# librosa/librosa

Measured on AMD Instinct MI355X. Metric: STFT+mel frames/sec (n_fft=2048 hop=512), higher is better.
Workload: dtype f32

## Files before the change

### librosa_amd/csrc/lra_api.hip

```cpp
#include <dlfcn.h>
#include <hip/hip_runtime.h>
#include <rocfft/rocfft.h>

#include <algorithm>
#include <atomic>
#include <chrono>
#include <cmath>
#include <cstdio>
#include <cstdlib>
#include <cstring>
#include <map>
#include <memory>
#include <mutex>
#include <string>
#include <thread>
#include <vector>

#include "../../include/librosa_amd.h"
#ifndef LRA_ISTFT16_DEFAULT
#define LRA_ISTFT16_DEFAULT 0
#endif
#ifndef LRA_V3_DEFAULT
#define LRA_V3_DEFAULT 1
#endif
// ... 46 lines not shown
    int opt_stft_iters = 0;
    int opt_istft_strip_groups = 0;
    int opt_variant = -1;
    int opt_autotune = 1;
    int opt_mel_runs = 1;
    int opt_mel_tile = 0;
    int opt_generic_mel = 0;
    int opt_lds_pad = 0;
    int opt_v2 = 1;
    int opt_istft16 = LRA_ISTFT16_DEFAULT;
    int opt_placement_retry = 0;
    struct PlacedAlloc {
        size_t padded = 0;
        std::vector<hipMemGenericAllocationHandle_t> handles;
        bool plain = false;
    };
    std::map<void*, PlacedAlloc> placed;
    std::mutex placed_mu;
    std::vector<std::pair<void*, size_t>> placed_retired;
    size_t placed_va_spent = 0;
    static constexpr size_t kPlacedVaBudget = (size_t)4 << 40;
    double placed_best_gbps = 0.0;
    int opt_v3 = LRA_V3_DEFAULT;
    int opt_mel_pc = LRA_MEL_PC_DEFAULT;
    int opt_mel_many = 1;
    int opt_cqt_merge = 1;
    int opt_hpss_tile = 1;
    int opt_mixed_inv_pow2 = 1;
    int opt_mixed_pow2_mel = 1;
    int opt_ola4 = 1;
    int opt_mixed_irfft = 1;
    int opt_mixed = 1;
    int opt_direct = 1;
    int opt_xcd_remap = 1;
    unsigned int* d_flag = nullptr;
    std::map<std::pair<int, int>, std::pair<void*, void*>> cqt_tw;
    std::string name;
    struct HostPipe* pipe = nullptr;
    hipStream_t side_stream = nullptr;
    hipStream_t side_main = nullptr;
    static constexpr int kForkRing = 16;
    hipEvent_t fork_event[kForkRing] = {}, side_passed[kForkRing] = {};
    bool fork_used[kForkRing] = {};
    int fork_next = 0;
    static constexpr int kJoinRing = 8;
    hipEvent_t join_event[kJoinRing] = {}, main_passed[kJoinRing] = {};
// ... 193 lines not shown
    if (it != cache.end()) return it->second;
    int per_cu = 0;
    if (lds > 65536) (void)hipFuncSetAttribute(kern, hipFuncAttributeMaxDynamicSharedMemorySize, lds);
    if (hipOccupancyMaxActiveBlocksPerMultiprocessor(&per_cu, kern, block, lds) != hipSuccess) per_cu = 0;
    (void)hipGetLastError();
    cache[key] = per_cu;
    return per_cu;
}

template <class T> struct StftLaunch {
    StftArgs<T> a;
    int mode = 0;
    long long batch = 0;
    int iters_opt = 0;
    int mel_tile_opt = 0;
    int n_cu = 256;
    void* out = nullptr;
    int lds_pad = 0;
    bool xcd_remap = true;
    bool use_v2 = true;
    bool use_direct = true;
    bool mel_v2 = false;
    bool mel_pc = false;
    bool mel_runs = true;
    const lra_mel_plan* mel = nullptr;
    hipStream_t stream = nullptr;
    hipError_t err = hipSuccess;

    template <class Cfg, int MODE> void launch(int shared_bytes) {
        static_assert(Cfg::P <= 4, "at most four Stockham passes are wired up");
        const int lds_probe_v1 = Cfg::FPB * stft_slot_bytes<Cfg>(MODE, a.n_mels, mel_tile_opt > 0 ? mel_tile_opt : 4) + shared_bytes + lds_pad;
        void (*kern)(StftArgs<T>, const T*, void*) = nullptr;
        bool direct = false;
        if constexpr (Cfg::PLAN == 0) {
        kern = stft_kernel<Cfg, MODE, POW_TWO, 0>;
        if (MODE != OUT_COMPLEX && a.power_mode == POW_ONE) kern = stft_kernel<Cfg, MODE, POW_ONE, 0>;
        if (MODE != OUT_COMPLEX && a.power_mode == POW_GENERAL) kern = stft_kernel<Cfg, MODE, POW_GENERAL, 0>;
        if constexpr (sizeof(T) == 4) {
#ifndef LRA_MEL_RA
#define LRA_MEL_RA 1
#endif
            if (ring_rows_aligned<Cfg>(a.hop) && (LRA_MEL_RA || MODE == OUT_COMPLEX || MODE == OUT_POWER)) {
                kern = stft_kernel<Cfg, MODE, POW_TWO, 1>;
                if (MODE != OUT_COMPLEX && a.power_mode == POW_ONE) kern = stft_kernel<Cfg, MODE, POW_ONE, 1>;
                if (MODE != OUT_COMPLEX && a.power_mode == POW_GENERAL) kern = stft_kernel<Cfg, MODE, POW_GENERAL, 1>;
            }
// ... 66 lines not shown
        if (lds > 160 * 1024) { err = hipErrorInvalidValue; return; }
        if (lds > 65536) {
            err = hipFuncSetAttribute(reinterpret_cast<const void*>(kern), hipFuncAttributeMaxDynamicSharedMemorySize, lds);
            if (err != hipSuccess) return;
        }
        a.n_blocks = (int)grid;
        a.xcd_chunk = (xcd_remap && grid >= 64) ? (int)((grid + 7) / 8) : 0;
        const long long launch_grid = a.xcd_chunk ? 8LL * a.xcd_chunk : grid;
        hipLaunchKernelGGL(kern, dim3((unsigned)launch_grid), dim3(Cfg::NT), lds, stream, a, a.y, out);
        err = hipGetLastError();
    }

    template <class Cfg> void launch_pc(int hd) {
        using PL = PcLayout<Cfg>;
        void (*kern)(StftArgs<T>, const T*, void*) = nullptr;
#define LRA_PICKP(HD)                                                        \
    kern = stft_pc_kernel<Cfg, HD, POW_TWO>;                                 \
    if (a.power_mode == POW_ONE) kern = stft_pc_kernel<Cfg, HD, POW_ONE>;    \
    if (a.power_mode == POW_GENERAL) kern = stft_pc_kernel<Cfg, HD, POW_GENERAL>;
        if (hd == 4) { LRA_PICKP(4) } else { LRA_PICKP(8) }
#undef LRA_PICKP
        const int lds = PL::BYTES + lds_pad;
        constexpr int fpb = PL::NP;
        int iters = iters_opt;
        if (iters <= 0) {
            const int per_cu = resident_workgroups(reinterpret_cast<const void*>(kern), PL::NT, lds);
            const long long conc = (long long)n_cu * (per_cu > 0 ? per_cu : 1);
            int best_iters = 0;
            double best_fill = -1.0;
            for (int cand = 176; cand >= 24; --cand) {
                const int wgpc = (a.n_frames + fpb * cand - 1) / (fpb * cand);
                const int it = (a.n_frames + fpb * wgpc - 1) / (fpb * wgpc);
                const double rounds = (double)(batch * wgpc) / (double)conc;
                const double fill = (rounds <= 1.0 && rounds >= 0.6) ? 1.0 : rounds / std::ceil(rounds);
                if (fill > best_fill + 0.02) { best_fill = fill; best_iters = it; }
            }
            iters = best_iters;
            while (iters > 4 && batch * ((a.n_frames + fpb * iters - 1) / (fpb * iters)) < 2LL * n_cu) iters /= 2;
        }
        if (iters < 1) iters = 1;
        a.rot_uniform = 0;
        a.mel_tile = 1;
        a.frames_per_wg = fpb * iters;
        a.wg_per_clip = (a.n_frames + a.frames_per_wg - 1) / a.frames_per_wg;
        a.slot_bytes = PL::FRAME;
        a.shared_off = 0;
        const long long grid = batch * a.wg_per_clip;
        if (grid > 0x7ffffff0LL) { err = hipErrorInvalidConfiguration; return; }
        a.n_blocks = (int)grid;
        a.xcd_chunk = (xcd_remap && grid >= 64) ? (int)((grid + 7) / 8) : 0;
        const long long launch_grid = a.xcd_chunk ? 8LL * a.xcd_chunk : grid;
        hipLaunchKernelGGL(kern, dim3((unsigned)launch_grid), dim3(PL::NT), lds, stream, a, a.y, out);
        err = hipGetLastError();
    }

    template <class Cfg> void operator()() {
        if constexpr (Cfg::REV) {
            err = hipErrorInvalidValue;
            return;
        } else if constexpr (Cfg::PLAN == 1) {
            if (!use_v2 || v2_hop_divisor<Cfg>(a.hop) == 0) { err = hipErrorInvalidValue; return; }
            if (mode == OUT_COMPLEX) launch<Cfg, OUT_COMPLEX>(0);
            else if (mode == OUT_POWER) launch<Cfg, OUT_POWER>(0);
            else if (mode == OUT_MEL2 && mel_pc && mel && mel->melr2_ok && mel_runs) {
                if constexpr (pc_cfg_ok<Cfg>()) {
                    const int hd_pc = v2_hop_divisor<Cfg>(a.hop);
                    if (!pc_bank_ok<Cfg>(a.n_mels, mel->melr2_pmax) || !pc_fits_budget<Cfg>(hd_pc, a.power_mode)) { err = hipErrorInvalidValue; return; }
                    a.melr_w = (const T*)mel->d_melr2_w;
                    a.melr_keep = (const T*)mel->d_melr2_keep;
                    a.melr_addr = mel->d_melr2_addr;
                    a.melr_zero = mel->melr2_zero;
                    a.melr_mid = mel->melr2_mid;
// ... 560 lines not shown
        L.out = out;
        L.a.power_mode = power_mode_of(power);
        L.a.power = (T)power;
        if (mel) {
            L.a.mel_c0 = mel->d_c0;
            L.a.mel_len = mel->d_len;
            L.a.mel_off = mel->d_off;
            L.a.mel_val = (const T*)mel->d_val;
            L.a.n_mels = mel->n_mels;
            L.a.mel_wAB = (const T*)mel->d_wAB;
            L.mel = mel;
        }
        L.a.nonfinite_flag = ctx->d_flag;
        L.mode = (mode == OUT_MEL && mel && mel->two_slope && !ctx->opt_generic_mel) ? OUT_MEL2 : mode;
        L.batch = batch;
        L.stream = ctx->stream;
        L.iters_opt = ctx->opt_stft_iters;
        L.n_cu = ctx->n_cu;
        L.mel_tile_opt = ctx->opt_mel_tile;
        L.lds_pad = ctx->opt_lds_pad;
        L.xcd_remap = ctx->opt_xcd_remap != 0;
        L.use_v2 = ctx->opt_v2 != 0;
        L.mel_pc = ctx->opt_mel_pc != 0;
        L.use_direct = ctx->opt_direct != 0;
        L.mel_runs = ctx->opt_mel_runs != 0;
        int variant = ctx->opt_variant >= 0 ? ctx->opt_variant : 0;
        auto launch = [&](int v) -> int {
            StftLaunch<T> Lv = L;
            Lv.a.tw = (const cx<T>*)p->d_tw[v];
            if (!dispatch_logm<T>(p->logm, v, Lv)) return fail(LRA_EINVAL, "unsupported power-of-two size");
            if (Lv.err != hipSuccess) return fail(LRA_EHIP, std::string("stft kernel launch: ") + hipGetErrorString(Lv.err));
            return LRA_OK;
        };
        bool v2_applies = false;
        if constexpr (sizeof(T) == 4)
            v2_applies = ctx->opt_v2 && (L.mode == OUT_COMPLEX || L.mode == OUT_POWER) && p->logm == 10 && v2_hop_divisor<typename CfgSel<float, 10, 0>::type>(p->hop) > 0;
        if (ctx->opt_variant < 0 && ctx->opt_autotune && sizeof(T) == 4 && p->logm == 10 && !v2_applies) {
            int& tuned = p->tuned_variant[L.mode & 3];
            if (tuned < 0 && batch * n_frames >= 65536) LRA_TRY(autotune_variant(ctx, launch, &tuned));
            if (tuned >= 0) variant = tuned;
        }
        bool pc_g = false;
        if constexpr (sizeof(T) == 4) {
            using C6 = typename CfgSel<float, 10, 6>::type;
            if (L.mode == OUT_MEL2 && ctx->opt_mel_pc == 2 && p->logm == 10 && mel && mel->melr2_ok && ctx->opt_mel_runs && ctx->opt_v2 && (ctx->opt_variant < 0 || ctx->opt_variant == 6))
                pc_g = pc_bank_ok<C6>(mel->n_mels, mel->melr2_pmax) && pc_fits_budget<C6>(v2_hop_divisor<C6>(p->hop), power_mode_of(power));
// ... 672 lines not shown
        return LRA_OK;
    }
    return fail(LRA_EINVAL, "lra_ctx_side: mode must be LRA_SIDE_FORK, LRA_SIDE_BACK, LRA_SIDE_JOIN or LRA_SIDE_END");
}

int lra_ctx_sync(lra_ctx* ctx) {
    LRA_BIND(ctx);
    LRA_HIP(hipStreamSynchronize(ctx->stream));
    return LRA_OK;
}

int lra_ctx_set_option(lra_ctx* ctx, const char* key, int value) {
    if (!ctx || !key) return fail(LRA_EINVAL, "null argument");
    if (!std::strcmp(key, "stft_iters")) ctx->opt_stft_iters = value;
    else if (!std::strcmp(key, "istft_strip_groups")) ctx->opt_istft_strip_groups = value;
    else if (!std::strcmp(key, "mel_tile")) ctx->opt_mel_tile = value;
    else if (!std::strcmp(key, "ablate")) (void)value;
    else if (!std::strcmp(key, "generic_mel")) ctx->opt_generic_mel = value;
    else if (!std::strcmp(key, "pipe_chunk_mb")) ctx->opt_pipe_chunk_mb = value > 0 ? value : 128;
    else if (!std::strcmp(key, "pipe_threads")) ctx->opt_pipe_threads = value > 0 ? value : 1;
    else if (!std::strcmp(key, "lds_pad")) ctx->opt_lds_pad = value;
    else if (!std::strcmp(key, "xcd_remap")) ctx->opt_xcd_remap = value != 0;
    else if (!std::strcmp(key, "v2")) ctx->opt_v2 = value != 0;
    else if (!std::strcmp(key, "mel_pc")) ctx->opt_mel_pc = (value == 1 || value == 2) ? value : 0;
    else if (!std::strcmp(key, "istft16")) ctx->opt_istft16 = value != 0;
    else if (!std::strcmp(key, "placement_retry")) ctx->opt_placement_retry = value < 0 ? 0 : (value > 8 ? 8 : value);
    else if (!std::strcmp(key, "v3")) ctx->opt_v3 = (value == 1 || value == 2) ? value : 0;
    else if (!std::strcmp(key, "cqt_merge")) ctx->opt_cqt_merge = value < 0 ? 0 : (value > 2 ? 2 : (int)value);
    else if (!std::strcmp(key, "mel_many")) ctx->opt_mel_many = value != 0;
    else if (!std::strcmp(key, "direct")) ctx->opt_direct = value != 0;
    else if (!std::strcmp(key, "mixed")) ctx->opt_mixed = value == 2 ? 2 : (value != 0);
    else if (!std::strcmp(key, "hpss_tile")) ctx->opt_hpss_tile = value != 0;
    else if (!std::strcmp(key, "mixed_pow2_mel")) ctx->opt_mixed_pow2_mel = value != 0;
    else if (!std::strcmp(key, "ola4")) ctx->opt_ola4 = value != 0;
    else if (!std::strcmp(key, "mixed_irfft")) ctx->opt_mixed_irfft = value != 0;
    else if (!std::strcmp(key, "mixed_inv_pow2")) ctx->opt_mixed_inv_pow2 = value != 0;
    else if (!std::strcmp(key, "autotune")) ctx->opt_autotune = value != 0;
    else if (!std::strcmp(key, "mel_runs")) ctx->opt_mel_runs = value != 0;
    else if (!std::strcmp(key, "variant")) ctx->opt_variant = (value >= 0 && value < kNumVariants) ? value : -1;
    else return fail(LRA_EINVAL, std::string("unknown option ") + key);
    return LRA_OK;
}

int lra_ctx_nonfinite_reset(lra_ctx* ctx) {
    LRA_BIND(ctx);
    LRA_HIP(hipMemsetAsync(ctx->d_flag, 0, sizeof(unsigned int), ctx->stream));
// ... 1763 lines not shown
```

### librosa_amd/csrc/lra_common.h

```cpp
#pragma once

#include <cstddef>
#include <cstdint>

#ifdef LRA_HOSTSIM
#include <cmath>
#include <cstdio>
#include <cstdlib>
#include <cstring>
#include <vector>
#define LRA_HD inline
#define LRA_UNROLL _Pragma("GCC unroll 64")
#else
#include <hip/hip_runtime.h>
#define LRA_HD __host__ __device__ __forceinline__
#define LRA_UNROLL _Pragma("unroll")
#endif

#ifndef LRA_NO_EXPECT
#define LRA_LIKELY(x) __builtin_expect(!!(x), 1)
#define LRA_UNLIKELY(x) __builtin_expect(!!(x), 0)
#else
#define LRA_LIKELY(x) (x)
#define LRA_UNLIKELY(x) (x)
// ... 248 lines not shown
};
inline State& state() { static thread_local State s; return s; }
}

struct Lds {
    size_t base;
};
template <class V> inline V lds_ld(Lds l, int byte_off) {
    auto& s = sim::state();
    s.note_read(l.base + byte_off, sizeof(V));
    V v; std::memcpy(&v, s.mem.data() + l.base + byte_off, sizeof(V)); return v;
}
template <class V> inline void lds_st(Lds l, int byte_off, V v) {
    auto& s = sim::state();
    s.note_write(l.base + byte_off, sizeof(V));
    std::memcpy(s.mem.data() + l.base + byte_off, &v, sizeof(V));
}
inline Lds lds_sub(Lds l, int byte_off) { Lds r; r.base = l.base + byte_off; return r; }

#define LRA_LAUNDER(p) ((void)0)
#define LRA_ATOMIC_OR(ptr, v) (*(ptr) |= (v))
#define LRA_UNIFORM(x) (x)
#define LRA_KEEP(x) ((void)0)
#define LRA_RAW_TID(tid) (tid)
template <class T> inline T fast_div(T x, T w) { return x / w; }
template <class V> inline void stream_store(V* p, V v) { *p = v; }
template <class V> inline void stream_store16(V* p, V v) { *p = v; }
template <class V> inline V stream_load(const V* p) { return *p; }
template <class T> inline void store4_unaligned(T* p, T a, T b, T c, T d) { p[0] = a; p[1] = b; p[2] = c; p[3] = d; }
#define LRA_PHASE(NT, tid) for (int tid = 0; tid < (NT); ++tid) { ::lra::sim::state().cur_tid = tid;
#define LRA_PHASE_END } ::lra::sim::state().barrier();
#define LRA_PHASE_END_SYNC(WAVE) } ::lra::sim::state().barrier(WAVE);
#define LRA_REGS(Type, name, NT) std::vector<Type> name##_all(NT)
#define LRA_R(name) name##_all[tid]
#define LRA_HALF_SWAP8(name, tid, first, active)                                                                  \
    if ((tid & 63) < 32 && (active)) {                                                                            \
        for (int m_ = 0; m_ < 8; ++m_) std::swap(name##_all[tid].v[(first) + m_], name##_all[tid + 32].v[(first) + m_]); \
    }

#else

struct Lds {
    char* base;
};
#ifndef LRA_LDS_NOMERGE
#define LRA_LDS_NOMERGE 1
#endif
template <class V> LRA_HD V lds_ld(Lds l, int byte_off) {
#if LRA_LDS_NOMERGE
    if constexpr (sizeof(V) == 8) {
        typedef float f2v __attribute__((ext_vector_type(2)));
        const f2v t = *(const volatile __attribute__((address_space(3))) f2v*)(l.base + byte_off);
        return __builtin_bit_cast(V, t);
    }
#endif
    return *reinterpret_cast<const V*>(l.base + byte_off);
}
template <class V> LRA_HD void lds_st(Lds l, int byte_off, V v) { *reinterpret_cast<V*>(l.base + byte_off) = v; }
LRA_HD Lds lds_sub(Lds l, int byte_off) { Lds r; r.base = l.base + byte_off; return r; }

#define LRA_LAUNDER(p) asm volatile("" : "+s"(p))
#define LRA_ATOMIC_OR(ptr, v) atomicOr((ptr), (v))
#define LRA_UNIFORM(x) __builtin_amdgcn_readfirstlane(x)
#define LRA_KEEP(x) asm volatile("" : "+v"(x))
#define LRA_RAW_TID(tid) ((int)threadIdx.x)
__device__ __forceinline__ float fast_div(float x, float w) { return x * __builtin_amdgcn_rcpf(w); }
__device__ __forceinline__ double fast_div(double x, double w) { return x / w; }
#ifndef LRA_NT_STORE
#define LRA_NT_STORE 0
#endif
template <class V> __device__ __forceinline__ void stream_store(V* p, V v) {
#if LRA_NT_STORE
    if constexpr (sizeof(V) == 8) {
        typedef float f2v __attribute__((ext_vector_type(2)));
        __builtin_nontemporal_store(__builtin_bit_cast(f2v, v), reinterpret_cast<f2v*>(p));
    } else if constexpr (sizeof(V) == 16) {
        typedef double d2v __attribute__((ext_vector_type(2)));
        __builtin_nontemporal_store(__builtin_bit_cast(d2v, v), reinterpret_cast<d2v*>(p));
    } else {
        __builtin_nontemporal_store(v, p);
    }
#else
    *p = v;
#endif
}
template <class T> __device__ __forceinline__ void store4_unaligned(T* p, T a, T b, T c, T d) {
    if constexpr (sizeof(T) == 4) {
// ... 77 lines not shown
```

### librosa_amd/csrc/lra_fused.h

```cpp
#pragma once

#include <hip/hip_runtime.h>

#include "lra_dispatch.h"
#include "lra_kernels_pc.h"

template <class Cfg, int MODE, int PM, int RA>
__global__ __launch_bounds__(Cfg::NT, Cfg::MIN_WAVES) void stft_kernel(lra::StftArgs<typename Cfg::real> a, const typename Cfg::real* __restrict__ y,
                                                                     void* __restrict__ out) {
    extern __shared__ __attribute__((aligned(16))) char lra_smem[];
    lra::Lds lds;
    lds.base = lra_smem;
    a.y = y;
    a.D = static_cast<typename Cfg::cplx*>(out);
    a.S = static_cast<typename Cfg::real*>(out);
    a.Mel = static_cast<typename Cfg::real*>(out);
    const int blk = lra::xcd_block((int)blockIdx.x, a.xcd_chunk);
    if (blk >= a.n_blocks) return;
    lra::stft_block<Cfg, MODE, PM, RA>(a, blk, lds);
}

#ifndef LRA_V3_WAVES
#define LRA_V3_WAVES 3
#endif
template <class Cfg, int HD, int MODE, int PM>
__global__ __launch_bounds__(Cfg::NT, (Cfg::NT > 256 ? 1 : (Cfg::TF == 64 && HD >= 4 && PM != lra::POW_GENERAL && MODE != lra::OUT_MELR ? (Cfg::PLAN == 1 ? LRA_V3_WAVES : 3) : 2))) void stft2_kernel(lra::StftArgs<typename Cfg::real> a, const typename Cfg::real* __restrict__ y,
                                                                                  void* __restrict__ out) {
    extern __shared__ __attribute__((aligned(16))) char lra_smem[];
    lra::Lds lds;
    lds.base = lra_smem;
    a.y = y;
    a.D = static_cast<typename Cfg::cplx*>(out);
    a.S = static_cast<typename Cfg::real*>(out);
    a.Mel = static_cast<typename Cfg::real*>(out);
    const int blk = lra::xcd_block((int)blockIdx.x, a.xcd_chunk);
    if (blk >= a.n_blocks) return;
    lra::stft_block2<Cfg, HD, MODE, PM>(a, blk, lds);
}

template <class Cfg, int HD, int PM>
__global__ __launch_bounds__(lra::PcLayout<Cfg>::NT, 3) void stft_pc_kernel(lra::StftArgs<typename Cfg::real> a, const typename Cfg::real* __restrict__ y, void* __restrict__ out) {
    extern __shared__ __attribute__((aligned(16))) char lra_smem[];
    lra::Lds lds;
    lds.base = lra_smem;
    a.y = y;
    a.Mel = static_cast<typename Cfg::real*>(out);
    const int blk = lra::xcd_block((int)blockIdx.x, a.xcd_chunk);
    if (blk >= a.n_blocks) return;
    lra::stft_pc_block<Cfg, HD, PM>(a, blk, lds);
}

template <class Cfg, int HC>
__global__ __launch_bounds__(Cfg::NT, Cfg::MIN_WAVES) void istft_kernel(lra::IstftArgs<typename Cfg::real> a, const typename Cfg::cplx* __restrict__ D,
                                                                      const typename Cfg::real* __restrict__ wss, typename Cfg::real* __restrict__ y) {
    extern __shared__ __attribute__((aligned(16))) char lra_smem[];
    lra::Lds lds;
    lds.base = lra_smem;
    a.D = D;
    a.wss = wss;
    a.y = y;
    const int blk = lra::xcd_block((int)blockIdx.x, a.xcd_chunk);
    if (blk >= a.n_blocks) return;
    lra::istft_block<Cfg, HC>(a, blk, lds);
}


namespace lra {

#define LRA_CFG_ALIAS(NAME, ...) using NAME = typename CfgSel<__VA_ARGS__>::type; using NAME##_mel = typename MelCfgOf<NAME>::type; using NAME##_melmany = typename MelManyCfgOf<NAME>::type;
LRA_CFG_ALIAS(cfg_f32_4, float, 4, 0)
LRA_CFG_ALIAS(cfg_f32_5, float, 5, 0)
// ... 85 lines not shown
```

### librosa_amd/csrc/lra_kernels.h

```cpp
#pragma once

#ifndef LRA_ABLATE
#define LRA_ABLATE 0
#endif

#include <cmath>
#include <limits>

#include "lra_fft.h"

#if defined(LRA_PHASE_TIMER) && !defined(LRA_HOSTSIM)
__device__ unsigned long long lra_phase_ticks[16];
#define LRA_TICK(i)                                                    \
    do {                                                               \
        const unsigned long long now__ = __builtin_amdgcn_s_memtime(); \
        tick_acc[i] += now__ - tick_prev;                              \
        tick_prev = now__;                                             \
    } while (0)
#define LRA_TICK_DECL unsigned long long tick_acc[16] = {}, tick_prev = __builtin_amdgcn_s_memtime()
#define LRA_TICK_FLUSH                                                                    \
    do {                                                                                  \
        if ((threadIdx.x & 63) == 0)                                                      \
            for (int i__ = 0; i__ < 16; ++i__) atomicAdd(&lra_phase_ticks[i__], tick_acc[i__]); \
    } while (0)
// ... 26 lines not shown
    cx<T>* D;
    T* S;
    long long row_pitch;
    T* Mel;
    int power_mode;
    T power;
    const int* mel_c0;
    const int* mel_len;
    const int* mel_off;
    const T* mel_val;
    int n_mels;
    const T* mel_wAB;
    const int* mel_run;
    const int* mel_segd;
    int mel_nyq;
    const T* melr_w;
    const T* melr_keep;
    const int* melr_addr;
    int rot_uniform;
    int melr_pmax;
    int melr_zero, melr_mid;
    int shared_off;
    int n_blocks, xcd_chunk;
    unsigned int* nonfinite_flag;
};

LRA_HD int xcd_block(int b, int chunk) { return chunk > 0 ? (b & 7) * chunk + (b >> 3) : b; }

template <class Cfg> LRA_HD int slot_of(int tid) {
    if (Cfg::FPB == 1) return 0;
    if (Cfg::TF >= 64) return LRA_UNIFORM((int)((unsigned)tid / (unsigned)Cfg::TF));
    return (int)((unsigned)tid / (unsigned)Cfg::TF);
}
template <class Cfg> LRA_HD int lane_of(int tid) { return (int)((unsigned)tid % (unsigned)Cfg::TF); }

#ifndef LRA_MELR_NB_SMALL
#define LRA_MELR_NB_SMALL 4
#endif
#ifndef LRA_MELR_PH_SMALL
#define LRA_MELR_PH_SMALL 3
#endif
constexpr int melr_nb_of_tf(int tf, bool many = false) { return tf >= 32 ? 2 : (many ? 8 : LRA_MELR_NB_SMALL); }
constexpr int melr_ph_of_tf(int tf, bool many = false) { return tf >= 32 ? 4 : (many ? 1 : LRA_MELR_PH_SMALL); }
template <class Cfg> constexpr bool melr_many() { return Cfg::TF == 16 && Cfg::NT == 128; }
template <class Cfg> constexpr int melr_nb() { return melr_nb_of_tf(Cfg::TF, melr_many<Cfg>()); }
template <class Cfg> constexpr int melr_ph() { return melr_ph_of_tf(Cfg::TF, melr_many<Cfg>()); }
// ... 1752 lines not shown
```

### librosa_amd/csrc/lra_kernels_pc.h

```cpp
#pragma once

#include "lra_kernels2.h"

namespace lra {

#ifndef LRA_PC_PRIO_PA
#define LRA_PC_PRIO_PA 3
#endif
#ifndef LRA_PC_PRIO_PS
#define LRA_PC_PRIO_PS 2
#endif
#ifndef LRA_PC_PRIO_CA
#define LRA_PC_PRIO_CA 0
#endif
#ifndef LRA_PC_PRIO_CB
#define LRA_PC_PRIO_CB 1
#endif
#ifndef LRA_PC_ROTATE
#define LRA_PC_ROTATE 1
#endif
#ifndef LRA_PC_SPIN_LIMIT
#define LRA_PC_SPIN_LIMIT (1 << 22)
#endif

// ... 79 lines not shown
    __builtin_amdgcn_fence(__ATOMIC_ACQUIRE, "wavefront");
}
__device__ __forceinline__ int pc_flag_load(Lds l, int off) { return *(const volatile __attribute__((address_space(3))) int*)(l.base + off); }
__device__ __forceinline__ void pc_flag_store(Lds l, int off, int v) { *(volatile __attribute__((address_space(3))) int*)(l.base + off) = v; }
__device__ __forceinline__ void pc_wait(Lds l, int off, int want, unsigned int* sticky) {
    int spins = 0;
    while (true) {
        const int v = LRA_UNIFORM(pc_flag_load(l, off));
        if (LRA_LIKELY(v >= want)) break;
        if (LRA_UNLIKELY(++spins > LRA_PC_SPIN_LIMIT)) {
            if (sticky && (threadIdx.x & 63) == 0) atomicOr(sticky, 2u);
            break;
        }
        __builtin_amdgcn_s_sleep(2);
    }
    pc_fence();
}
__device__ __forceinline__ void pc_wait_ready(Lds l, int off, int want, unsigned int* sticky) {
    if (LRA_UNLIKELY(LRA_UNIFORM(pc_flag_load(l, off)) < want)) pc_wait(l, off, want, sticky);
    else pc_fence();
}
#endif

template <class Cfg, int HD> LRA_HD void pc_producer_prologue(const StftArgs<typename Cfg::real>& a, int clip, int frame0, int tf, Regs2<Cfg, HD>& rg) {
    using T = typename Cfg::real;
    if constexpr (Cfg::PLAN == 1) v3_hoist<Cfg, HD>(rg, tf, a.win, a.tw, a.twr);
    else v2_hoist<Cfg, HD>(rg, tf, a.win, a.tw, a.twr);
    v2_fill<Cfg, HD>(a, clip, frame0, tf, rg);
    if constexpr (v2_rotate_asm_ok<Cfg, HD>() && LRA_PC_ROTATE) {
        LRA_UNROLL
        for (int e = 0; e < Cfg::R; ++e) { LRA_KEEP(rg.raw[e].x); LRA_KEEP(rg.raw[e].y); }
    }
    LRA_UNROLL
    for (int e = 0; e < Regs2<Cfg, HD>::NEW; ++e) rg.pf[e] = mk<T>((T)0, (T)0);
}
template <class Cfg, int HD> LRA_HD void pc_producer_pass0(const StftArgs<typename Cfg::real>& a, int clip, int frame, int it, bool more, int tf, Regs2<Cfg, HD>& rg, Lds fr) {
    if (v2_rotate_asm_ok<Cfg, HD>() && LRA_PC_ROTATE) {
        v2_window_rotating<Cfg, HD>(it, rg);
        if (more) v2_issue_loads<Cfg, HD>(a, clip, frame + 1, tf, rg);
        v2_pass0_dft<Cfg, HD>(tf, rg, fr);
    } else {
        if (it > 0) v2_shift<Cfg, HD>(rg);
        if (more) v2_issue_loads<Cfg, HD>(a, clip, frame + 1, tf, rg);
        v2_pass0<Cfg, HD>(frame < a.n_frames, tf, rg, fr);
    }
}

template <class Cfg, int p> LRA_HD void pc_mid_dft_write(typename Cfg::cplx* v, const typename Cfg::cplx* treg, Lds fr, int tf) {
    if constexpr (Cfg::PLAN == 1) {
        v3_mid_twiddle_dft<Cfg>(v, treg);
        v3_mid_write<Cfg>(v, fr, tf);
    } else {
        pass_twiddle_dft_reg<Cfg, p>(v, treg);
        pass_write<Cfg, p>(v, fr, tf);
    }
}
template <class Cfg, int HD> LRA_HD void pc_last_read(Regs2<Cfg, HD>& rg, Lds fr, int tf) {
    if constexpr (Cfg::PLAN == 1) v3_last_read<Cfg, HD>(rg, fr, tf);
    else v2_last_read<Cfg, HD>(rg, fr, tf);
}
template <class Cfg, int HD, int PM> LRA_HD void pc_last_power_row(const StftArgs<typename Cfg::real>& a, int clip, int frame, int tf, Regs2<Cfg, HD>& rg, Lds pwr) {
    if constexpr (Cfg::PLAN == 1) v3_last_split_store<Cfg, HD, OUT_MELR, PM, false>(a, clip, frame, frame < a.n_frames, tf, rg, pwr);
    else v2_last_split_store<Cfg, HD, OUT_MELR, PM, false, false>(a, clip, frame, frame < a.n_frames, tf, rg, pwr);
}

template <class Cfg> LRA_HD void pc_consumer_prologue(const StftArgs<typename Cfg::real>& a, int clip, int f_first, int iters, int tf, PcRegs<Cfg>& rg, Lds wg) {
    using T = typename Cfg::real;
    using C = typename Cfg::cplx;
    using RG = PcRegs<Cfg>;
    constexpr int BPL = Cfg::R / 2, TF = Cfg::TF;
    const C* __restrict__ w2 = reinterpret_cast<const C*>(a.melr_w);
    LRA_UNROLL
    for (int run = 0; run < 2; ++run) {
        LRA_UNROLL
        for (int j = 0; j < BPL; ++j) rg.w[run * BPL + j] = w2[BPL * (run * TF + tf) + j];
    }
    rg.wq = w2[Cfg::M];
    LRA_UNROLL
    for (int jj = 0; jj < Cfg::R; ++jj) rg.keep[jj] = a.melr_keep[jj * TF + tf];
    LRA_UNROLL
    for (int b = 0; b < RG::NB; ++b) {
        const int m = RG::NB * tf + b;
        LRA_UNROLL
        for (int h = 0; h < 2; ++h) {
            LRA_UNROLL
            for (int q = 0; q < RG::PH; ++q) {
                const int ad = PcLayout<Cfg>::rs_off() + (m < a.n_mels ? a.melr_addr[(h * a.melr_pmax + q) * a.n_mels + m] : a.melr_zero);
                rg.mad[b][h * RG::PH + q] = pc_mad_addr(wg, ad & ~(2 * (int)sizeof(T) - 1));
            }
        }
    }
    LRA_UNROLL
    for (int run = 0; run < 2; ++run) {
        const int first = 8 * (run * TF + tf);
        rg.pwa[2 * run] = v2_pw_index<Cfg>(first) * (int)sizeof(T);
        rg.pwa[2 * run + 1] = v2_pw_index<Cfg>(first + 4) * (int)sizeof(T);
    }
    rg.pwx = (tf == 0 ? v2_pw_index<Cfg>(Cfg::M) : 0) * (int)sizeof(T);
    LRA_UNROLL
    for (int b = 0; b < RG::NB; ++b) {
        const int m = RG::NB * tf + b;
        rg.row[b] = a.Mel + ((long long)clip * a.n_mels + (m < a.n_mels ? m : 0)) * a.n_frames;
    }
    LRA_UNROLL
    for (int s = 0; s < RG::NP; ++s) {
        LRA_UNROLL
        for (int b = 0; b < RG::NB; ++b) {
            rg.ph[s][b] = LRA_MEL_ALIGNED_BURSTS ? (int)(((long long)clip * a.n_mels * a.n_frames + (long long)b * a.n_frames + f_first + s * iters) & (RG::TILE - 1)) : 0;
            LRA_UNROLL
            for (int k = 0; k < RG::TILE; ++k) rg.mt[s][RG::TILE * b + k] = (T)0;
        }
    }
    rg.pw_extra = (T)0;
}
template <class Cfg> LRA_HD void pc_runs_read(PcRegs<Cfg>& rg, Lds pwr) {
    using T = typename Cfg::real;
    constexpr int BPL = Cfg::R / 2;
    static_assert(BPL == 8, "runs of 8 bins");
    LRA_UNROLL
    for (int run = 0; run < 2; ++run) {
        const V4<T> lo = lds_ld<V4<T>>(pwr, rg.pwa[2 * run]), hi = lds_ld<V4<T>>(pwr, rg.pwa[2 * run + 1]);
        T* d = rg.pw + run * BPL;
        d[0] = lo.a; d[1] = lo.b; d[2] = lo.c; d[3] = lo.d; d[4] = hi.a; d[5] = hi.b; d[6] = hi.c; d[7] = hi.d;
    }
    rg.pw_extra = lds_ld<T>(pwr, rg.pwx);
}
template <class Cfg> LRA_HD void pc_accumulate(const StftArgs<typename Cfg::real>& a, int tf, PcRegs<Cfg>& rg, Lds rs) {
    using T = typename Cfg::real;
    using C = typename Cfg::cplx;
    constexpr int BPL = Cfg::R / 2, TF = Cfg::TF;
    LRA_UNROLL
    for (int run = 0; run < 2; ++run) {
        C acc = mk<T>((T)0, (T)0);
        LRA_UNROLL
        for (int j = 0; j < BPL; ++j) {
            const int jj = run * BPL + j;
// ... 31 lines not shown
            LRA_UNROLL
            for (int q = 0; q < PH; ++q) acc += x[b][h * PH + q];
            part[h] = acc;
        }
        const T v = part[0] + part[1];
        int s8;
        if constexpr (UNI) {
            s8 = (rg.ph[S][b] + it) & (MT - 1);
            mt[MT * b + s8] = v;
        } else {
            s8 = (int)((rg.row[b] - a.Mel + frame) & (MT - 1));
            LRA_UNROLL
            for (int k = 0; k < MT; ++k) mt[MT * b + k] = k == s8 ? v : mt[MT * b + k];
        }
        if (last_of_slot || s8 == MT - 1) {
            T t8[MT];
            pc_tile_band(mt, b, t8);
            melr_burst_row(rg.row[b] + (frame - s8), s8, it, t8);
        }
    }
    return mt;
}

#ifndef LRA_HOSTSIM
template <class Cfg, bool UNI> __device__ __forceinline__ void pc_consumer(const StftArgs<typename Cfg::real>& a, int clip, int f_first, int iters, int n_it, Lds lds) {
    using L = PcLayout<Cfg>;
    constexpr int TF = Cfg::TF;
    PcRegs<Cfg> rg;
    const Lds rs = lds_sub(lds, L::rs_off());
    const int tf = (int)(threadIdx.x & (TF - 1));
    pc_consumer_prologue<Cfg>(a, clip, f_first, iters, tf, rg, lds);
    pc_fence();
    for (int it = 0; it < n_it; ++it) {
#define LRA_PC_SERVE(S)                                                                                                        \
        {                                                                                                                      \
            const int frame = f_first + S * iters + it;                                                                       \
            v2_setprio<LRA_PC_PRIO_CA>();                                                                                      \
            pc_wait_ready(lds, L::ready_off(S), it + 1, a.nonfinite_flag);                                                     \
            pc_runs_read<Cfg>(rg, lds_sub(lds, L::pw_off(S)));                                                                 \
            pc_fence();                                                                                                        \
            if (tf == 0) pc_flag_store(lds, L::consumed_off(S), it + 1);                             \
            pc_fence();                                                                                                        \
            pc_accumulate<Cfg>(a, tf, rg, rs);                                                                                 \
            pc_fence();                                                                                                        \
            v2_setprio<LRA_PC_PRIO_CB>();                                                                                      \
            if (frame < a.n_frames) rg.mt[S] = pc_combine<Cfg, S, UNI>(a, clip, frame, tf, it, it + 1 == iters || frame + 1 >= a.n_frames, rg, lds, rg.mt[S]); \
            pc_fence();                                                                                                        \
        }
        LRA_PC_SERVE(0)
        LRA_PC_SERVE(1)
#undef LRA_PC_SERVE
    }
}
#endif

template <class Cfg, int HD, int PM = POW_TWO> LRA_HD void stft_pc_block(const StftArgs<typename Cfg::real>& a_in, const int blk, Lds lds) {
    static_assert(pc_cfg_ok<Cfg>(), "producer / consumer mel kernel: one wave per frame, mirrored last pass, swizzled power row");
    using T = typename Cfg::real;
    using L = PcLayout<Cfg>;
    using RG = Regs2<Cfg, HD>;
    constexpr int NP = L::NP, TF = Cfg::TF;
    StftArgs<T> a = a_in;
    const int clip = blk / a.wg_per_clip;
    const int f_first = (blk % a.wg_per_clip) * a.frames_per_wg;
    const int iters = a.frames_per_wg / NP;
    const int left = a.n_frames - f_first;
    const int n_it = left < iters ? left : iters;
#ifdef LRA_HOSTSIM
    LRA_REGS(RG, prg, L::NT);
    LRA_REGS(PcRegs<Cfg>, crg, L::NT);
    LRA_PHASE(L::NT, tid) {
        const int w = tid / TF, tf = tid % TF;
        if (w < NP) pc_producer_prologue<Cfg, HD>(a, clip, f_first + w * iters, tf, LRA_R(prg));
        else pc_consumer_prologue<Cfg>(a, clip, f_first, iters, tf, LRA_R(crg), lds);
        if (tid < 2 * NP) pc_flag_store(lds, L::flags_off() + 4 * tid, 0);
    } LRA_PHASE_END
    for (int it = 0; it < n_it; ++it) {
        LRA_PHASE(L::NT, tid) {
            const int w = tid / TF, tf = tid % TF;
            if (w < NP) pc_producer_pass0<Cfg, HD>(a, clip, f_first + w * iters + it, it, it + 1 < iters, tf, LRA_R(prg), lds_sub(lds, L::frame_off(w)));
        } LRA_PHASE_END_SYNC(true)
#define LRA_PC_MID(p)                                                                                                                   \
        if (Cfg::P - 1 > p) {                                                                                                           \
            LRA_PHASE(L::NT, tid) {                                                                                                     \
                if (tid / TF < NP) pass_read<Cfg, (p < Cfg::P ? p : 0)>(LRA_R(prg).v, lds_sub(lds, L::frame_off(tid / TF)), tid % TF);  \
            } LRA_PHASE_END_SYNC(true)                                                                                                  \
            LRA_PHASE(L::NT, tid) {                                                                                                     \
                if (tid / TF < NP) pc_mid_dft_write<Cfg, (p < Cfg::P ? p : 0)>(LRA_R(prg).v, LRA_R(prg).treg, lds_sub(lds, L::frame_off(tid / TF)), tid % TF); \
            } LRA_PHASE_END_SYNC(true)                                                                                                  \
        }
        LRA_PC_MID(1)
        LRA_PC_MID(2)
#undef LRA_PC_MID
        LRA_PHASE(L::NT, tid) {
            if (tid / TF < NP) pc_last_read<Cfg, HD>(LRA_R(prg), lds_sub(lds, L::frame_off(tid / TF)), tid % TF);
        } LRA_PHASE_END_SYNC(true)
        LRA_PHASE(L::NT, tid) {
            const int w = tid / TF, tf = tid % TF, frame = f_first + w * iters + it;
            if (w < NP) pc_last_power_row<Cfg, HD, PM>(a, clip, frame, tf, LRA_R(prg), lds_sub(lds, L::pw_off(w)));
        } LRA_PHASE_END
        for (int s = 0; s < NP; ++s) {
            LRA_PHASE(L::NT, tid) {
                if (tid / TF == NP) pc_runs_read<Cfg>(LRA_R(crg), lds_sub(lds, L::pw_off(s)));
            } LRA_PHASE_END_SYNC(true)
            LRA_PHASE(L::NT, tid) {
                if (tid / TF == NP) pc_accumulate<Cfg>(a, tid % TF, LRA_R(crg), lds_sub(lds, L::rs_off()));
            } LRA_PHASE_END_SYNC(true)
            LRA_PHASE(L::NT, tid) {
                const int tf = tid % TF, frame = f_first + s * iters + it;
                if (tid / TF == NP && frame < a.n_frames) {
                    const bool last = it + 1 == iters || frame + 1 >= a.n_frames;
                    if (pc_tile_uniform<Cfg>(a)) {
                        if (s == 0) LRA_R(crg).mt[0] = pc_combine<Cfg, 0, true>(a, clip, frame, tf, it, last, LRA_R(crg), lds, LRA_R(crg).mt[0]);
                        else LRA_R(crg).mt[1] = pc_combine<Cfg, 1, true>(a, clip, frame, tf, it, last, LRA_R(crg), lds, LRA_R(crg).mt[1]);
                    } else {
                        if (s == 0) LRA_R(crg).mt[0] = pc_combine<Cfg, 0, false>(a, clip, frame, tf, it, last, LRA_R(crg), lds, LRA_R(crg).mt[0]);
                        else LRA_R(crg).mt[1] = pc_combine<Cfg, 1, false>(a, clip, frame, tf, it, last, LRA_R(crg), lds, LRA_R(crg).mt[1]);
                    }
                }
            } LRA_PHASE_END_SYNC(true)
        }
        sim::state().barrier();
    }
#else
    if (threadIdx.x < 2 * NP) pc_flag_store(lds, L::flags_off() + 4 * (int)threadIdx.x, 0);
    phase_sync<false>();
    const int wave = LRA_UNIFORM((int)(threadIdx.x / TF));
    if (wave < NP) {
        RG rg;
        const Lds fr = lds_sub(lds, L::frame_off(wave)), pwr = lds_sub(lds, L::pw_off(wave));
        {
            const int tf = phase_tid() % TF;
            pc_producer_prologue<Cfg, HD>(a, clip, f_first + wave * iters, tf, rg);
        }
        pc_fence();
        for (int it = 0; it < n_it; ++it) {
            const int frame = f_first + wave * iters + it;
            v2_setprio<LRA_PC_PRIO_PA>();
            {
                const int tf = phase_tid() % TF;
                pc_producer_pass0<Cfg, HD>(a, clip, frame, it, it + 1 < iters, tf, rg, fr);
            }
            pc_fence();
#define LRA_PC_MID(p)                                                                                    \
            if (Cfg::P - 1 > p) {                                                                        \
                { const int tf = phase_tid() % TF; pass_read<Cfg, (p < Cfg::P ? p : 0)>(rg.v, fr, tf); } \
                pc_fence();                                                                              \
                { const int tf = phase_tid() % TF; pc_mid_dft_write<Cfg, (p < Cfg::P ? p : 0)>(rg.v, rg.treg, fr, tf); } \
                pc_fence();                                                                              \
            }
            LRA_PC_MID(1)
            LRA_PC_MID(2)
#undef LRA_PC_MID
            int taken;
            {
                const int tf = phase_tid() % TF;
                pc_last_read<Cfg, HD>(rg, fr, tf);
                taken = pc_flag_load(lds, L::consumed_off(wave));
            }
            pc_fence();
            v2_setprio<LRA_PC_PRIO_PS>();
            if (LRA_UNLIKELY(LRA_UNIFORM(taken) < it)) pc_wait(lds, L::consumed_off(wave), it, a.nonfinite_flag);
            {
                const int tf = phase_tid() % TF;
                pc_last_power_row<Cfg, HD, PM>(a, clip, frame, tf, rg, pwr);
            }
            pc_fence();
            if (phase_tid() % TF == 0) pc_flag_store(lds, L::ready_off(wave), it + 1);
            pc_fence();
        }
    } else {
        if (pc_tile_uniform<Cfg>(a)) pc_consumer<Cfg, true>(a, clip, f_first, iters, n_it, lds);
        else pc_consumer<Cfg, false>(a, clip, f_first, iters, n_it, lds);
    }
#endif
}

}
```

Measured before the change: 639.1 million.

## Make producer-consumer mel STFT kernel persistent over a grid-stride work loop

The producer/consumer mel kernel now launches at most as many workgroups as can be resident (or a user-set pc_grid) and loops over strip items with a grid stride. Window, twiddle and filterbank loads are hoisted out of the per-item setup so they are done once per workgroup, and the ready/consumed handshake counters keep running across items. The aim is to cut launch tail and repeated prologue cost, at the price of more complex flag accounting and possible load imbalance when items do not divide evenly across workgroups.

```diff
diff --git a/librosa_amd/csrc/lra_api.hip b/librosa_amd/csrc/lra_api.hip
--- a/librosa_amd/csrc/lra_api.hip
+++ b/librosa_amd/csrc/lra_api.hip
@@ -92,6 +92,7 @@
     static constexpr size_t kPlacedVaBudget = (size_t)4 << 40;
     double placed_best_gbps = 0.0;
     int opt_v3 = LRA_V3_DEFAULT;
+    int opt_pc_grid = 0;
     int opt_mel_pc = LRA_MEL_PC_DEFAULT;
     int opt_mel_many = 1;
     int opt_cqt_merge = 1;
@@ -331,6 +332,7 @@
     bool use_direct = true;
     bool mel_v2 = false;
     bool mel_pc = false;
+    int pc_grid = 0;
     bool mel_runs = true;
     const lra_mel_plan* mel = nullptr;
     hipStream_t stream = nullptr;
@@ -443,10 +445,10 @@
 #undef LRA_PICKP
         const int lds = PL::BYTES + lds_pad;
         constexpr int fpb = PL::NP;
+        const int per_cu = resident_workgroups(reinterpret_cast<const void*>(kern), PL::NT, lds);
+        const long long conc = (long long)n_cu * (per_cu > 0 ? per_cu : 1);
         int iters = iters_opt;
         if (iters <= 0) {
-            const int per_cu = resident_workgroups(reinterpret_cast<const void*>(kern), PL::NT, lds);
-            const long long conc = (long long)n_cu * (per_cu > 0 ? per_cu : 1);
             int best_iters = 0;
             double best_fill = -1.0;
             for (int cand = 176; cand >= 24; --cand) {
@@ -466,9 +468,12 @@
         a.wg_per_clip = (a.n_frames + a.frames_per_wg - 1) / a.frames_per_wg;
         a.slot_bytes = PL::FRAME;
         a.shared_off = 0;
-        const long long grid = batch * a.wg_per_clip;
-        if (grid > 0x7ffffff0LL) { err = hipErrorInvalidConfiguration; return; }
-        a.n_blocks = (int)grid;
+        const long long items = batch * a.wg_per_clip;
+        if (items > 0x7ffffff0LL) { err = hipErrorInvalidConfiguration; return; }
+        long long grid = items < conc ? items : conc;
+        if (pc_grid > 0) grid = items < pc_grid ? items : pc_grid;
+        a.n_blocks = (int)items;
+        a.n_wg = (int)grid;
         a.xcd_chunk = (xcd_remap && grid >= 64) ? (int)((grid + 7) / 8) : 0;
         const long long launch_grid = a.xcd_chunk ? 8LL * a.xcd_chunk : grid;
         hipLaunchKernelGGL(kern, dim3((unsigned)launch_grid), dim3(PL::NT), lds, stream, a, a.y, out);
@@ -1075,6 +1080,7 @@
         L.xcd_remap = ctx->opt_xcd_remap != 0;
         L.use_v2 = ctx->opt_v2 != 0;
         L.mel_pc = ctx->opt_mel_pc != 0;
+        L.pc_grid = ctx->opt_pc_grid;
         L.use_direct = ctx->opt_direct != 0;
         L.mel_runs = ctx->opt_mel_runs != 0;
         int variant = ctx->opt_variant >= 0 ? ctx->opt_variant : 0;
@@ -1793,6 +1799,7 @@
     else if (!std::strcmp(key, "lds_pad")) ctx->opt_lds_pad = value;
     else if (!std::strcmp(key, "xcd_remap")) ctx->opt_xcd_remap = value != 0;
     else if (!std::strcmp(key, "v2")) ctx->opt_v2 = value != 0;
+    else if (!std::strcmp(key, "pc_grid")) ctx->opt_pc_grid = value > 0 ? value : 0;
     else if (!std::strcmp(key, "mel_pc")) ctx->opt_mel_pc = (value == 1 || value == 2) ? value : 0;
     else if (!std::strcmp(key, "istft16")) ctx->opt_istft16 = value != 0;
     else if (!std::strcmp(key, "placement_retry")) ctx->opt_placement_retry = value < 0 ? 0 : (value > 8 ? 8 : value);
diff --git a/librosa_amd/csrc/lra_common.h b/librosa_amd/csrc/lra_common.h
--- a/librosa_amd/csrc/lra_common.h
+++ b/librosa_amd/csrc/lra_common.h
@@ -294,6 +294,7 @@
 #define LRA_ATOMIC_OR(ptr, v) (*(ptr) |= (v))
 #define LRA_UNIFORM(x) (x)
 #define LRA_KEEP(x) ((void)0)
+#define LRA_KEEP_SCALAR(x) ((void)0)
 #define LRA_RAW_TID(tid) (tid)
 template <class T> inline T fast_div(T x, T w) { return x / w; }
 template <class V> inline void stream_store(V* p, V v) { *p = v; }
@@ -335,6 +336,7 @@
 #define LRA_ATOMIC_OR(ptr, v) atomicOr((ptr), (v))
 #define LRA_UNIFORM(x) __builtin_amdgcn_readfirstlane(x)
 #define LRA_KEEP(x) asm volatile("" : "+v"(x))
+#define LRA_KEEP_SCALAR(x) asm volatile("" : "+s"(x))
 #define LRA_RAW_TID(tid) ((int)threadIdx.x)
 __device__ __forceinline__ float fast_div(float x, float w) { return x * __builtin_amdgcn_rcpf(w); }
 __device__ __forceinline__ double fast_div(double x, double w) { return x / w; }
diff --git a/librosa_amd/csrc/lra_fused.h b/librosa_amd/csrc/lra_fused.h
--- a/librosa_amd/csrc/lra_fused.h
+++ b/librosa_amd/csrc/lra_fused.h
@@ -46,7 +46,7 @@
     a.y = y;
     a.Mel = static_cast<typename Cfg::real*>(out);
     const int blk = lra::xcd_block((int)blockIdx.x, a.xcd_chunk);
-    if (blk >= a.n_blocks) return;
+    if (blk >= a.n_wg) return;
     lra::stft_pc_block<Cfg, HD, PM>(a, blk, lds);
 }
 
diff --git a/librosa_amd/csrc/lra_kernels.h b/librosa_amd/csrc/lra_kernels.h
--- a/librosa_amd/csrc/lra_kernels.h
+++ b/librosa_amd/csrc/lra_kernels.h
@@ -72,6 +72,7 @@
     int melr_zero, melr_mid;
     int shared_off;
     int n_blocks, xcd_chunk;
+    int n_wg;
     unsigned int* nonfinite_flag;
 };
 
diff --git a/librosa_amd/csrc/lra_kernels_pc.h b/librosa_amd/csrc/lra_kernels_pc.h
--- a/librosa_amd/csrc/lra_kernels_pc.h
+++ b/librosa_amd/csrc/lra_kernels_pc.h
@@ -125,10 +125,12 @@
 }
 #endif
 
-template <class Cfg, int HD> LRA_HD void pc_producer_prologue(const StftArgs<typename Cfg::real>& a, int clip, int frame0, int tf, Regs2<Cfg, HD>& rg) {
-    using T = typename Cfg::real;
+template <class Cfg, int HD> LRA_HD void pc_producer_hoist(const StftArgs<typename Cfg::real>& a, int tf, Regs2<Cfg, HD>& rg) {
     if constexpr (Cfg::PLAN == 1) v3_hoist<Cfg, HD>(rg, tf, a.win, a.tw, a.twr);
     else v2_hoist<Cfg, HD>(rg, tf, a.win, a.tw, a.twr);
+}
+template <class Cfg, int HD> LRA_HD void pc_producer_item(const StftArgs<typename Cfg::real>& a, int clip, int frame0, int tf, Regs2<Cfg, HD>& rg) {
+    using T = typename Cfg::real;
     v2_fill<Cfg, HD>(a, clip, frame0, tf, rg);
     if constexpr (v2_rotate_asm_ok<Cfg, HD>() && LRA_PC_ROTATE) {
         LRA_UNROLL
@@ -167,7 +169,7 @@
     else v2_last_split_store<Cfg, HD, OUT_MELR, PM, false, false>(a, clip, frame, frame < a.n_frames, tf, rg, pwr);
 }
 
-template <class Cfg> LRA_HD void pc_consumer_prologue(const StftArgs<typename Cfg::real>& a, int clip, int f_first, int iters, int tf, PcRegs<Cfg>& rg, Lds wg) {
+template <class Cfg> LRA_HD void pc_consumer_hoist(const StftArgs<typename Cfg::real>& a, int tf, PcRegs<Cfg>& rg, Lds wg) {
     using T = typename Cfg::real;
     using C = typename Cfg::cplx;
     using RG = PcRegs<Cfg>;
@@ -179,8 +181,6 @@
         for (int j = 0; j < BPL; ++j) rg.w[run * BPL + j] = w2[BPL * (run * TF + tf) + j];
     }
     rg.wq = w2[Cfg::M];
-    LRA_UNROLL
-    for (int jj = 0; jj < Cfg::R; ++jj) rg.keep[jj] = a.melr_keep[jj * TF + tf];
     LRA_UNROLL
     for (int b = 0; b < RG::NB; ++b) {
         const int m = RG::NB * tf + b;
@@ -200,6 +200,16 @@
         rg.pwa[2 * run + 1] = v2_pw_index<Cfg>(first + 4) * (int)sizeof(T);
     }
     rg.pwx = (tf == 0 ? v2_pw_index<Cfg>(Cfg::M) : 0) * (int)sizeof(T);
+    rg.pw_extra = (T)0;
+#ifndef LRA_HOSTSIM
+    __builtin_amdgcn_sched_barrier(0);
+#endif
+    LRA_UNROLL
+    for (int jj = 0; jj < Cfg::R; ++jj) rg.keep[jj] = a.melr_keep[jj * TF + tf];
+}
+template <class Cfg> LRA_HD void pc_consumer_item(const StftArgs<typename Cfg::real>& a, int clip, int f_first, int iters, int tf, PcRegs<Cfg>& rg) {
+    using T = typename Cfg::real;
+    using RG = PcRegs<Cfg>;
     LRA_UNROLL
     for (int b = 0; b < RG::NB; ++b) {
         const int m = RG::NB * tf + b;
@@ -214,7 +224,6 @@
             for (int k = 0; k < RG::TILE; ++k) rg.mt[s][RG::TILE * b + k] = (T)0;
         }
     }
-    rg.pw_extra = (T)0;
 }
 template <class Cfg> LRA_HD void pc_runs_read(PcRegs<Cfg>& rg, Lds pwr) {
     using T = typename Cfg::real;
@@ -292,34 +301,64 @@
     return mt;
 }
 
-#ifndef LRA_HOSTSIM
-template <class Cfg, bool UNI> __device__ __forceinline__ void pc_consumer(const StftArgs<typename Cfg::real>& a, int clip, int f_first, int iters, int n_it, Lds lds) {
+struct PcItem {
+    int clip, f_first, n_it;
+};
+template <class T> LRA_HD PcItem pc_item(const StftArgs<T>& a, int i, int iters) {
+    PcItem w;
+    w.clip = LRA_UNIFORM(i / a.wg_per_clip);
+    w.f_first = (i - w.clip * a.wg_per_clip) * a.frames_per_wg;
+    const int left = a.n_frames - w.f_first;
+    w.n_it = left < iters ? left : iters;
+    return w;
+}
+
+#ifdef LRA_HOSTSIM
+inline int pc_sim_env(const char* name) {
+    const char* e = std::getenv(name);
+    return e ? std::atoi(e) : 0;
+}
+inline void pc_sim_expect(Lds l, int off, int want) {
+    if (pc_flag_load(l, off) < want) {
+        if (std::getenv("LRA_SIM_DEBUG")) std::fprintf(stderr, "hostsim: hand-over count at %d below %d\n", off, want);
+        ++sim::state().races;
+    }
+}
+#else
+template <class Cfg, bool UNI> __device__ __forceinline__ void pc_consumer(const StftArgs<typename Cfg::real>& a, int first, int n_items, int stride, int iters, Lds lds) {
     using L = PcLayout<Cfg>;
     constexpr int TF = Cfg::TF;
     PcRegs<Cfg> rg;
     const Lds rs = lds_sub(lds, L::rs_off());
     const int tf = (int)(threadIdx.x & (TF - 1));
-    pc_consumer_prologue<Cfg>(a, clip, f_first, iters, tf, rg, lds);
-    pc_fence();
-    for (int it = 0; it < n_it; ++it) {
+    pc_consumer_hoist<Cfg>(a, tf, rg, lds);
+    int done = 0;
+    for (int item = first; item < n_items; item += stride) {
+        const PcItem w = pc_item(a, item, iters);
+        const int clip = w.clip, f_first = w.f_first, n_it = w.n_it;
+        pc_consumer_item<Cfg>(a, clip, f_first, iters, phase_tid() & (TF - 1), rg);
+        pc_fence();
+        for (int it = 0; it < n_it; ++it) {
 #define LRA_PC_SERVE(S)                                                                                                        \
-        {                                                                                                                      \
-            const int frame = f_first + S * iters + it;                                                                       \
-            v2_setprio<LRA_PC_PRIO_CA>();                                                                                      \
-            pc_wait_ready(lds, L::ready_off(S), it + 1, a.nonfinite_flag);                                                     \
-            pc_runs_read<Cfg>(rg, lds_sub(lds, L::pw_off(S)));                                                                 \
-            pc_fence();                                                                                                        \
-            if (tf == 0) pc_flag_store(lds, L::consumed_off(S), it + 1);                             \
-            pc_fence();                                                                                                        \
-            pc_accumulate<Cfg>(a, tf, rg, rs);                                                                                 \
-            pc_fence();                                                                                                        \
-            v2_setprio<LRA_PC_PRIO_CB>();                                                                                      \
-            if (frame < a.n_frames) rg.mt[S] = pc_combine<Cfg, S, UNI>(a, clip, frame, tf, it, it + 1 == iters || frame + 1 >= a.n_frames, rg, lds, rg.mt[S]); \
-            pc_fence();                                                                                                        \
-        }
-        LRA_PC_SERVE(0)
-        LRA_PC_SERVE(1)
+            {                                                                                                                  \
+                const int frame = f_first + S * iters + it;                                                                   \
+                v2_setprio<LRA_PC_PRIO_CA>();                                                                                  \
+                pc_wait_ready(lds, L::ready_off(S), done + it + 1, a.nonfinite_flag);                                          \
+                pc_runs_read<Cfg>(rg, lds_sub(lds, L::pw_off(S)));                                                             \
+                pc_fence();                                                                                                    \
+                if (tf == 0) pc_flag_store(lds, L::consumed_off(S), done + it + 1);                  \
+                pc_fence();                                                                                                    \
+                pc_accumulate<Cfg>(a, tf, rg, rs);                                                                             \
+                pc_fence();                                                                                                    \
+                v2_setprio<LRA_PC_PRIO_CB>();                                                                                  \
+                if (frame < a.n_frames) rg.mt[S] = pc_combine<Cfg, S, UNI>(a, clip, frame, tf, it, it + 1 == iters || frame + 1 >= a.n_frames, rg, lds, rg.mt[S]); \
+                pc_fence();                                                                                                    \
+            }
+            LRA_PC_SERVE(0)
+            LRA_PC_SERVE(1)
 #undef LRA_PC_SERVE
+        }
+        done += n_it;
     }
 }
 #endif
@@ -331,20 +370,30 @@
     using RG = Regs2<Cfg, HD>;
     constexpr int NP = L::NP, TF = Cfg::TF;
     StftArgs<T> a = a_in;
-    const int clip = blk / a.wg_per_clip;
-    const int f_first = (blk % a.wg_per_clip) * a.frames_per_wg;
     const int iters = a.frames_per_wg / NP;
-    const int left = a.n_frames - f_first;
-    const int n_it = left < iters ? left : iters;
 #ifdef LRA_HOSTSIM
+    const int sim_grid = pc_sim_env("LRA_SIM_PC_GRID");
+    const int stride = sim_grid > 0 ? sim_grid : 1;
+    const int n_items = sim_grid > 0 ? pc_sim_env("LRA_SIM_PC_ITEMS") : blk + 1;
+    if (sim_grid > 0 && n_items <= 0) { std::fprintf(stderr, "hostsim: LRA_SIM_PC_GRID needs LRA_SIM_PC_ITEMS (batch x strips per clip)\n"); std::abort(); }
+    if (sim_grid > 0 && blk >= sim_grid) return;
     LRA_REGS(RG, prg, L::NT);
     LRA_REGS(PcRegs<Cfg>, crg, L::NT);
     LRA_PHASE(L::NT, tid) {
         const int w = tid / TF, tf = tid % TF;
-        if (w < NP) pc_producer_prologue<Cfg, HD>(a, clip, f_first + w * iters, tf, LRA_R(prg));
-        else pc_consumer_prologue<Cfg>(a, clip, f_first, iters, tf, LRA_R(crg), lds);
+        if (w < NP) pc_producer_hoist<Cfg, HD>(a, tf, LRA_R(prg));
+        else pc_consumer_hoist<Cfg>(a, tf, LRA_R(crg), lds);
         if (tid < 2 * NP) pc_flag_store(lds, L::flags_off() + 4 * tid, 0);
     } LRA_PHASE_END
+    int done = 0;
+    for (int item = blk; item < n_items; item += stride) {
+    const PcItem wi = pc_item(a, item, iters);
+    const int clip = wi.clip, f_first = wi.f_first, n_it = wi.n_it;
+    LRA_PHASE(L::NT, tid) {
+        const int w = tid / TF, tf = tid % TF;
+        if (w < NP) pc_producer_item<Cfg, HD>(a, clip, f_first + w * iters, tf, LRA_R(prg));
+        else pc_consumer_item<Cfg>(a, clip, f_first, iters, tf, LRA_R(crg));
+    } LRA_PHASE_END_SYNC(true)
     for (int it = 0; it < n_it; ++it) {
         LRA_PHASE(L::NT, tid) {
             const int w = tid / TF, tf = tid % TF;
@@ -363,15 +412,25 @@
         LRA_PC_MID(2)
 #undef LRA_PC_MID
         LRA_PHASE(L::NT, tid) {
-            if (tid / TF < NP) pc_last_read<Cfg, HD>(LRA_R(prg), lds_sub(lds, L::frame_off(tid / TF)), tid % TF);
+            if (tid / TF < NP) {
+                pc_last_read<Cfg, HD>(LRA_R(prg), lds_sub(lds, L::frame_off(tid / TF)), tid % TF);
+                if (tid % TF == 0) pc_sim_expect(lds, L::consumed_off(tid / TF), done + it);
+            }
         } LRA_PHASE_END_SYNC(true)
         LRA_PHASE(L::NT, tid) {
             const int w = tid / TF, tf = tid % TF, frame = f_first + w * iters + it;
-            if (w < NP) pc_last_power_row<Cfg, HD, PM>(a, clip, frame, tf, LRA_R(prg), lds_sub(lds, L::pw_off(w)));
+            if (w < NP) {
+                pc_last_power_row<Cfg, HD, PM>(a, clip, frame, tf, LRA_R(prg), lds_sub(lds, L::pw_off(w)));
+                if (tf == 0) pc_flag_store(lds, L::ready_off(w), done + it + 1);
+            }
         } LRA_PHASE_END
         for (int s = 0; s < NP; ++s) {
             LRA_PHASE(L::NT, tid) {
-                if (tid / TF == NP) pc_runs_read<Cfg>(LRA_R(crg), lds_sub(lds, L::pw_off(s)));
+                if (tid / TF == NP) {
+                    if (tid % TF == 0) pc_sim_expect(lds, L::ready_off(s), done + it + 1);
+                    pc_runs_read<Cfg>(LRA_R(crg), lds_sub(lds, L::pw_off(s)));
+                    if (tid % TF == 0) pc_flag_store(lds, L::consumed_off(s), done + it + 1);
+                }
             } LRA_PHASE_END_SYNC(true)
             LRA_PHASE(L::NT, tid) {
                 if (tid / TF == NP) pc_accumulate<Cfg>(a, tid % TF, LRA_R(crg), lds_sub(lds, L::rs_off()));
@@ -392,7 +451,10 @@
         }
         sim::state().barrier();
     }
+    done += n_it;
+    }
 #else
+    const int n_items = a.n_blocks, stride = a.n_wg;
     if (threadIdx.x < 2 * NP) pc_flag_store(lds, L::flags_off() + 4 * (int)threadIdx.x, 0);
     phase_sync<false>();
     const int wave = LRA_UNIFORM((int)(threadIdx.x / TF));
@@ -401,11 +463,19 @@
         const Lds fr = lds_sub(lds, L::frame_off(wave)), pwr = lds_sub(lds, L::pw_off(wave));
         {
             const int tf = phase_tid() % TF;
-            pc_producer_prologue<Cfg, HD>(a, clip, f_first + wave * iters, tf, rg);
+            pc_producer_hoist<Cfg, HD>(a, tf, rg);
+        }
+        int item = blk, cnt = 0, it = 0;
+        PcItem w = pc_item(a, item, iters);
+        int clip = w.clip, f0 = w.f_first + wave * iters, n_it = w.n_it;
+        {
+            const int tf = phase_tid() % TF;
+            pc_producer_item<Cfg, HD>(a, clip, f0, tf, rg);
         }
         pc_fence();
-        for (int it = 0; it < n_it; ++it) {
-            const int frame = f_first + wave * iters + it;
+        while (true) {
+            LRA_KEEP_SCALAR(cnt);
+            const int frame = f0 + it;
             v2_setprio<LRA_PC_PRIO_PA>();
             {
                 const int tf = phase_tid() % TF;
@@ -430,20 +500,32 @@
             }
             pc_fence();
             v2_setprio<LRA_PC_PRIO_PS>();
-            if (LRA_UNLIKELY(LRA_UNIFORM(taken) < it)) pc_wait(lds, L::consumed_off(wave), it, a.nonfinite_flag);
+            if (LRA_UNLIKELY(LRA_UNIFORM(taken) < cnt)) pc_wait(lds, L::consumed_off(wave), cnt, a.nonfinite_flag);
             {
                 const int tf = phase_tid() % TF;
                 pc_last_power_row<Cfg, HD, PM>(a, clip, frame, tf, rg, pwr);
             }
             pc_fence();
-            if (phase_tid() % TF == 0) pc_flag_store(lds, L::ready_off(wave), it + 1);
+            ++cnt;
+            if (phase_tid() % TF == 0) pc_flag_store(lds, L::ready_off(wave), cnt);
             pc_fence();
+            if (LRA_UNLIKELY(++it == n_it)) {
+                item += stride;
+                if (item >= n_items) break;
+                w = pc_item(a, item, iters);
+                clip = w.clip, f0 = w.f_first + wave * iters, n_it = w.n_it, it = 0;
+                {
+                    const int tf = phase_tid() % TF;
+                    pc_producer_item<Cfg, HD>(a, clip, f0, tf, rg);
+                }
+                pc_fence();
+            }
         }
     } else {
-        if (pc_tile_uniform<Cfg>(a)) pc_consumer<Cfg, true>(a, clip, f_first, iters, n_it, lds);
-        else pc_consumer<Cfg, false>(a, clip, f_first, iters, n_it, lds);
-    }
-#endif
-}
-
-}
+        if (pc_tile_uniform<Cfg>(a)) pc_consumer<Cfg, true>(a, blk, n_items, stride, iters, lds);
+        else pc_consumer<Cfg, false>(a, blk, n_items, stride, iters, lds);
+    }
+#endif
+}
+
+}
```

Result: no change. 638.2 million (-0.1%).
